# Tzq2doc/distributed_learning_simulator

Hardware: AMD Instinct MI355X
Metric: FL rounds/sec (FedAvg, 100 clients, ResNet-18, CIFAR-10-shaped) (higher is better)
Workload: dtype fp32; 1 GPU; fedavg_resnet18; model=ResNet18, algo=fed_avg, clients=100, local_epochs=5, global_batch=6400, per_client_batch=64, parallelism=client-dp1, backend=hip

## Files before the change

### csrc/bindings.cpp

```cpp
#include <pybind11/pybind11.h>

#include <stdexcept>
#include <string>

#include "dls.h"

namespace py = pybind11;
typedef uintptr_t ptr;

template <typename T>
static T* P(ptr p) {
  return reinterpret_cast<T*>(p);
}
static hipStream_t S(ptr s) { return reinterpret_cast<hipStream_t>(s); }

extern "C" const char* dls_src_hash();

static SgdEpi sgd_arg(const py::object& o) {
  SgdEpi e{};
  if (o.is_none()) return e;
  const py::tuple t = o.cast<py::tuple>();
  if (t.size() != 13) throw std::invalid_argument("sgd epilogue: 13 fields expected");
  e.theta = P<float>(t[0].cast<ptr>());
  e.mom = P<float>(t[1].cast<ptr>());
// ... 37 lines not shown
    p.stats = P<float>(stats);
    p.stats_valid = P<const int>(stats_valid);
    p.f32 = f32;
    p.ldx = ldx;
    p.ldy = ldy;
    p.acc = P<const bf16_t>(acc);
    p.gate = P<const bf16_t>(gate);
    p.x = P<const bf16_t>(x);
    p.w = P<const bf16_t>(w);
    p.y = P<bf16_t>(y);
    p.bias = P<const bf16_t>(bias);
    p.x_cs = x_cs; p.y_cs = y_cs; p.w_cs = w_cs; p.b_cs = b_cs;
    p.B = B; p.H = H; p.W = W; p.C = C; p.OH = OH; p.OW = OW; p.KH = KH; p.KW = KW;
    p.stride = stride; p.pad = pad; p.dil = dil; p.M = M; p.N = N; p.R = R; p.rep = rep; p.relu = relu;
    p.b_kmajor = b_kmajor;
    if (stats && stats_valid && native_option(g_opt_halo_skip, "DLS_SKIP_INVALID", 1)) {
      p.skip_valid = P<const int>(stats_valid);
      p.skip_mul = OH * OW;
    }
    conv_nt(p, K, variant, S(s));
  });
  m.def("conv_dgrad", [](ptr dy, ptr w, ptr dx, ptr acc, long w_cs, int K, int rep, int B, int OH, int OW, int Co, int H,
                         int W, int Ci, int KH, int KW, int stride, int pad, int variant, int f32, ptr s, int ld_dy,
                         long dy_cs, ptr wsplit, long ws_cs, long ws_plane, long x_lo, int acc_compact, ptr bnb_part,
                         ptr bnb_x, long bnb_xld, ptr bnb_y, ptr bnb_mask, ptr bnb_mean, ptr bnb_rstd, ptr bnb_valid,
                         ptr wt_buf, ptr acc_mask, int wt_ready) {
    BNBwdPartials bnb{P<float>(bnb_part), P<const float>(bnb_x), bnb_xld, P<const float>(bnb_y),
                      P<const uint8_t>(bnb_mask), P<const float>(bnb_mean), P<const float>(bnb_rstd),
                      P<const int>(bnb_valid)};
    conv_dgrad(P<const bf16_t>(dy), P<const bf16_t>(w), P<bf16_t>(dx), P<const bf16_t>(acc), w_cs, K, rep, B, OH, OW, Co, H, W, Ci, KH, KW,
               stride, pad, variant, f32, S(s), ld_dy, dy_cs, P<const bf16_t>(wsplit), ws_cs, ws_plane, x_lo, acc_compact,
               bnb_part ? &bnb : nullptr, P<bf16_t>(wt_buf), P<const uint8_t>(acc_mask), wt_ready);
  });
  m.def("wt_planes", [](ptr wsplit, long ws_cs, long ws_plane, ptr wt, int Kw, int Co, int Ci, ptr s) {
    wt_planes(P<const bf16_t>(wsplit), ws_cs, ws_plane, P<bf16_t>(wt), Kw, Co, Ci, S(s));
  });
  m.def("conv_gl_wanted", &conv_gl_wanted);
  m.def("conv_gl_fwd", [](ptr x, ptr w, ptr y, ptr bias, long x_cs, long y_cs, long w_cs, long b_cs, int K, int rep,
                          int B, int H, int W, int C, int OH, int OW, int KH, int KW, int stride, int pad, int N,
                          int relu, ptr s) {
    conv_gl_fwd(P<const bf16_t>(x), P<const bf16_t>(w), P<bf16_t>(y), P<const bf16_t>(bias), x_cs, y_cs, w_cs, b_cs,
                K, rep, B, H, W, C, OH, OW, KH, KW, stride, pad, N, relu, S(s));
  });
  m.def("conv_weight_flip_t", [](ptr w, ptr wt, long w_cs, int Kw, int Co, int KH, int KW, int Ci, ptr s) {
    conv_weight_flip_t(P<const bf16_t>(w), P<bf16_t>(wt), w_cs, Kw, Co, KH, KW, Ci, S(s));
  });
  m.def("conv_gl_dgrad", [](ptr dy, ptr wt, ptr dx, ptr acc, int K, int rep, int B, int OH, int OW, int Co, int H, int W,
                            int Ci, int KH, int KW, int stride, int pad, ptr s) {
    conv_gl_dgrad(P<const bf16_t>(dy), P<const bf16_t>(wt), P<bf16_t>(dx), P<const bf16_t>(acc), K, rep, B, OH, OW, Co, H, W, Ci, KH, KW,
                  stride, pad, S(s));
  });
  m.def("conv_nt_num_variants", &conv_nt_num_variants);
  m.def("conv_nt_default_variant", &conv_nt_default_variant);
  m.def("conv_tn_bn_bwd", [](ptr dy, ptr x, ptr dw, long x_cs, long dw_cs, int B, int H, int W, int C, int OH, int OW,
                             int KH, int KW, int stride, int pad, int M, int Co, int R, int K, int variant, ptr s,
                             int ldx, ptr part, ptr bn_x, ptr bn_mask, ptr bn_coef, ptr bn_valid) {
    ConvTNParams p{};
    p.part = P<float>(part);
    p.f32 = 1;
    p.ldy = Co;
    p.ldx = ldx;
    p.dy = P<const bf16_t>(dy);
    p.x = P<const bf16_t>(x);
    p.dw = P<float>(dw);
    p.dy_cs = (long)M * Co; p.x_cs = x_cs; p.dw_cs = dw_cs;
    p.B = B; p.H = H; p.W = W; p.C = C; p.OH = OH; p.OW = OW; p.KH = KH; p.KW = KW; p.stride = stride; p.pad = pad;
// ... 456 lines not shown
```

### csrc/conv_nt.hip

```cpp
#include "dls.h"
#include "gemm_common.h"

#include <numeric>

namespace {

template <int BM, int BN, int BK, int WM, int WN, int VA, int VB, bool BKM, int DEPTH>
__global__ void __launch_bounds__(WM* WN * 64) conv_nt_kernel(ConvNTParams p) {
  constexpr int T = WM * WN * 64;
  constexpr int TM = BM / (WM * 32);
  constexpr int TN = BN / (WN * 32);
  constexpr int LDA = BK + 8;
  constexpr int KCA = BK / VA, RPA = T / KCA, PA = BM / RPA;
  constexpr int KCB = BK / VB, RPB = T / KCB, PB = BN / RPB;
  constexpr int CCB = BN / VB, RPK = T / CCB, PK = BK / RPK;
  constexpr int LDBK = BN + 32;
  constexpr int NB = BKM ? PK : PB;
  static_assert(PA >= 1 && NB >= 1, "tile too small for thread count");
  static_assert(TM >= 1 && TN >= 1, "wave tile");
  constexpr int NBUF = DEPTH == 0 ? 1 : 2;
  constexpr int B_ROWS = BKM ? BK : BN, B_COLS = BKM ? LDBK : LDA;
  constexpr int A_BYTES = NBUF * BM * LDA * 2, B_BYTES = NBUF * B_ROWS * B_COLS * 2;
  constexpr int SW = TN * 32 + 8;
  constexpr int EPI_BYTES = WM * WN * 32 * SW * 2;
// ... 346 lines not shown
  p.fd_ohw = make_fastdiv((uint32_t)(p.OH * p.OW));
  p.fd_ow = make_fastdiv((uint32_t)p.OW);
  p.fd_kwc = make_fastdiv((uint32_t)(p.KW * p.C));
  p.fd_c = make_fastdiv((uint32_t)p.C);
  if (p.f32) {
    conv_nt_f32(p, K, variant, s);
    return;
  }
  if (p.stats) {
    fprintf(stderr, "conv_nt: epilogue statistics need the fp32 kernels\n");
    abort();
  }
  const bool bkm = p.b_kmajor != 0;
  int va = vec_width(std::gcd(p.C, p.ldx));
  int vb = bkm ? vec_width(p.N) : vec_width(p.R);
  if (va == 1 && vb == 4) vb = 1;
  if (variant < 0) {
    variant = conv_nt_default_variant(p.M, p.N, p.R, p.b_kmajor);
    (void)K;
  }
  const bool w84 = (va == 8 || va == 4) && (vb == 8 || vb == 4);
  if (w84 && !(va == 8 && vb == 8) && !(variant == 0 || variant == 10 || variant == 13 || variant == 6 ||
                                        variant == 7 || variant == 18)) {
    variant = (p.N <= 64) ? 13 : (bkm ? 10 : 0);
  } else if (!w84 && !(variant == 6 || variant == 7 || variant == 18)) {
    variant = (p.N <= 64) ? 7 : 6;
  }
  if (!launch_variant(variant, p, K, va, vb, bkm, s)) fprintf(stderr, "conv_nt: bad variant %d\n", variant);
}

void wt_planes(const bf16_t* wsplit, long ws_cs, long ws_plane, bf16_t* wt, int Kw, int Co, int Ci, hipStream_t s) {
  hipLaunchKernelGGL(wt_planes_kernel, dim3(Kw * 2 * 9, Co / 32, Ci / 32), dim3(256), 0, s, wsplit, ws_cs, ws_plane, wt,
                     Co, Ci);
}

void conv_dgrad(const bf16_t* dy, const bf16_t* w, bf16_t* dx, const bf16_t* acc, long w_cs, int K, int rep, int B, int OH, int OW,
                int Co, int H, int W, int Ci, int KH, int KW, int stride, int pad, int variant, int f32, hipStream_t s,
                int ld_dy, long dy_cs, const bf16_t* wsplit, long ws_cs, long ws_plane, long x_lo, int acc_compact,
                const BNBwdPartials* bnb, bf16_t* wt_buf, const uint8_t* acc_mask, int wt_ready) {
  ConvNTParams p{};
  p.acc_mask = acc_mask;
  if (bnb) {
    if (!f32 || stride != 1 || Ci % 4 != 0 || (bnb->mask && Ci % 8 != 0) || (bnb->xld && bnb->xld % 4 != 0)) {
      fprintf(stderr, "conv_dgrad: BN-backward partials need an fp32 stride-1 dgrad with Ci %% 4 == 0\n");
      abort();
    }
    p.bnb = bnb->part;
    p.bnb_x = bnb->x;
    p.bnb_xld = bnb->xld ? bnb->xld : Ci;
    p.bnb_y = bnb->y;
    p.bnb_mask = bnb->mask;
    p.bnb_mean = bnb->mean;
    p.bnb_rstd = bnb->rstd;
    p.bnb_valid = bnb->valid;
    if (stride == 1 && bnb->valid && native_option(g_opt_halo_skip, "DLS_SKIP_INVALID", 1)) {
      p.skip_valid = bnb->valid;
      p.skip_mul = 1;
    }
  }
  p.x_lo = x_lo;
  p.wsplit = wsplit;
  p.ws_cs = ws_cs;
  p.ws_plane = ws_plane;
  p.f32 = f32;
  p.ldx = ld_dy;
  p.x = dy;
// ... 16 lines not shown
  p.wKH = KH;
  p.wKW = KW;
  p.dil = 1;
  p.stride = 1;
  if (stride == 1) {
    p.OH = H;
    p.OW = W;
    p.KH = KH;
    p.KW = KW;
    p.pad = KH - 1 - pad;
    p.pad_w = KW - 1 - pad;
    p.kh_off = KH - 1;
    p.kw_off = KW - 1;
    p.kh_step = p.kw_step = 1;
    p.out_s = 1;
    p.M = B * H * W;
    p.R = KH * KW * Co;
    if (variant < 0 && !f32 && Ci <= 64 && vec_width(Ci) == 8 && vec_width(Co) == 8) variant = 14;
    if (wt_buf && f32 && x_lo != 0 && wsplit && KH == 3 && KW == 3 && pad == 1 && Co % 32 == 0 && Ci % 32 == 0) {
      const int Kw = K / rep;
      if (!wt_ready)
        hipLaunchKernelGGL(wt_planes_kernel, dim3(Kw * 2 * 9, Co / 32, Ci / 32), dim3(256), 0, s, wsplit, ws_cs,
                           ws_plane, wt_buf, Co, Ci);
      p.b_kmajor = 0;
      p.wsplit = wt_buf;
      p.ws_cs = 2L * 9 * Ci * Co;
      p.ws_plane = 9L * Ci * Co;
      p.w = wt_buf;
      p.w_cs = p.ws_cs;
    }
    conv_nt(p, K, variant, s);
    return;
  }
  for (int ph = 0; ph < stride; ++ph) {
    const int Hc = (H - ph + stride - 1) / stride;
    if (Hc <= 0) continue;
    const int kh0 = (ph + pad) % stride;
    const int nkh = kh0 < KH ? (KH - kh0 + stride - 1) / stride : 0;
    const int dh = (ph + pad - kh0) / stride;
    for (int pw = 0; pw < stride; ++pw) {
      const int Wc = (W - pw + stride - 1) / stride;
      if (Wc <= 0) continue;
      const int kw0 = (pw + pad) % stride;
      const int nkw = kw0 < KW ? (KW - kw0 + stride - 1) / stride : 0;
      const int dw = (pw + pad - kw0) / stride;
      ConvNTParams q = p;
      q.OH = Hc;
      q.OW = Wc;
      q.M = B * Hc * Wc;
      if (acc_compact) {
        q.acc = (ph == 0 && pw == 0) ? acc : nullptr;
        q.acc_compact = 1;
        q.acc_cs = (long)B * Hc * Wc * Ci;
      }
      q.out_s = stride;
      q.out_ph = ph;
      q.out_pw = pw;
      q.out_H = H;
      q.out_W = W;
      if (nkh == 0 || nkw == 0) {
        q.KH = q.KW = 1;
        q.R = 0;
        q.pad = q.pad_w = 0;
        q.kh_off = q.kw_off = 0;
        q.kh_step = q.kw_step = 1;
      } else {
// ... 14 lines not shown
```

### csrc/dls.h

```cpp
#pragma once
#include <hip/hip_runtime.h>
#include <stdint.h>

typedef uint16_t bf16_t;

constexpr int kOptUnset = -1000000;
extern int g_opt_attn_mfma, g_opt_conv_gl, g_opt_pl_min_wg;
extern int g_opt_halo_wgrad_unroll;
extern int g_opt_halo_skip;
extern int g_opt_conv_pix;
int native_option(int& slot, const char* env, int dflt);
bool set_native_option(const char* name, int value);

struct FastDiv {
  uint32_t d, mul, shift;
};

static inline FastDiv make_fastdiv(uint32_t d) {
  FastDiv f;
  f.d = d;
  uint32_t s = 0;
  while ((1u << s) < d) ++s;
  f.shift = s;
  f.mul = (uint32_t)((((uint64_t)1 << 32) * (((uint64_t)1 << s) - d)) / d + 1);
  return f;
}

__device__ __forceinline__ uint32_t fdiv(uint32_t n, const FastDiv& f) {
  return (__umulhi(n, f.mul) + n) >> f.shift;
}

struct ConvNTParams {
  const bf16_t* x;
  const bf16_t* w;
  bf16_t* y;
  const bf16_t* bias;
  const bf16_t* acc;
  long acc_cs;
  int acc_compact;
  const uint8_t* acc_mask;
  const bf16_t* gate;
  long x_cs, y_cs, w_cs, b_cs;
  int B, H, W, C;
// ... 173 lines not shown
void conv_gl_fwd(const bf16_t* x, const bf16_t* w, bf16_t* y, const bf16_t* bias, long x_cs, long y_cs, long w_cs,
                 long b_cs, int K, int rep, int B, int H, int W, int C, int OH, int OW, int KH, int KW, int stride,
                 int pad, int N, int relu, hipStream_t s);
void conv_weight_flip_t(const bf16_t* w, bf16_t* wt, long w_cs, int Kw, int Co, int KH, int KW, int Ci,
                        hipStream_t s);
void conv_gl_dgrad(const bf16_t* dy, const bf16_t* wt, bf16_t* dx, const bf16_t* acc, int K, int rep, int B, int OH, int OW, int Co,
                   int H, int W, int Ci, int KH, int KW, int stride, int pad, hipStream_t s);

void conv_nt(ConvNTParams p, int K, int variant, hipStream_t s);
int conv_nt_num_variants();
int conv_nt_default_variant(int M, int N, int R, int b_kmajor);
void conv_dgrad(const bf16_t* dy, const bf16_t* w, bf16_t* dx, const bf16_t* acc, long w_cs, int K, int rep, int B, int OH, int OW,
                int Co, int H, int W, int Ci, int KH, int KW, int stride, int pad, int variant, int f32, hipStream_t s,
                int ld_dy = 0, long dy_cs = 0, const bf16_t* wsplit = nullptr, long ws_cs = 0, long ws_plane = 0,
                long x_lo = 0, int acc_compact = 0,
                const BNBwdPartials* bnb = nullptr,
                bf16_t* wt_buf = nullptr,
                const uint8_t* acc_mask = nullptr,
                int wt_ready = 0);
void wt_planes(const bf16_t* wsplit, long ws_cs, long ws_plane, bf16_t* wt, int Kw, int Co, int Ci, hipStream_t s);
void conv_tn(ConvTNParams p, int K, int variant, hipStream_t s);
int conv_tn_num_variants();
int conv_tn_splitk(int K, int Co, int R, int M, int C, int variant, int f32, int ldy = 0, int ldx = 0,
                   int planes = 0);
void conv_nt_f32(const ConvNTParams& p, int K, int variant, hipStream_t s);
int conv_nt_f32_num_variants();
void conv_tn_f32(ConvTNParams p, int K, int variant, hipStream_t s);
bool conv_nt_pl_supported(const ConvNTParams& p);
bool conv_nt_pl(const ConvNTParams& p, int K, int variant, hipStream_t s);
int conv_nt_pl_num_variants();
int conv_nt_pl_variant();
void conv_nt_pl_set_variant(int v);
bool conv_halo(const ConvNTParams& p, int K, hipStream_t s);
bool conv_halo_bn_supported(int B, int H, int W, int C, int N);
void bn_coef_sums(const double* sums, long sums_cs, int ldp, const float* gamma, const float* beta,
                  const int* valid_rows, long g_cs, int K, int R, int C, float eps, int rep, float* mean, float* rstd,
                  float* coef, hipStream_t s);
void part_sum_f64(const float* part, int K, int nparts, int g, double* out, long out_cs, int ldo, hipStream_t s);
long chan_sums_f64_ws(int R, int C);
void chan_sums_f64(const float* x, long x_cs, int ldx, int K, int R, int C, const int* valid, double* ws, double* out,
                   long out_cs, int ldo, hipStream_t s);
void bn_apply_only(const float* x, const float* coef, const int* valid_rows, int K, int R, int C, int relu,
                   bf16_t* yp, uint8_t* rmask, hipStream_t s, float* y = nullptr);
bool conv_halo_bn_fwd(const float* x, long x_cs, const float* coef, int relu, const int* valid_rows,
                      const bf16_t* wsplit, long ws_cs, long ws_plane, int rep, float* y, long y_cs, int K, int B,
                      int H, int W, int C, int N, float* stats, const int* stats_valid, hipStream_t s,
                      bf16_t* yp = nullptr, uint8_t* mask = nullptr);
bool conv_halo_bn_dense_supported(int B, int H, int W, int C, int N);
bool conv_halo_bn_dense_fwd(const float* x, long x_cs, int ldx, int creal, const float* coef, int relu,
                            const int* valid_rows, const bf16_t* wsplit, long ws_cs, long ws_plane, int rep, float* y,
                            long y_cs, int ldy, int K, int B, int H, int W, int C, int N, float* stats,
                            const int* stats_valid, float* ny, long ny_cs, int ldny, uint8_t* mask, hipStream_t s);
bool dense_dgrad_supported(int B, int H, int W, int C, int N);
long dense_dgrad_ws_floats(int K, int B, int H, int C);
bool dense_dgrad_bn(DenseDgradParams p, const float* gamma, long g_cs, float* dgamma, float* dbeta, long dg_cs,
                    float* ws, hipStream_t s);
void bn_bwd_coef_parts(const float* part, int nparts, const float* gamma, long g_cs, const int* valid_rows,
                       const float* mean, const float* rstd, int K, int R, int C, float* coef, float* dgamma,
                       float* dbeta, long dg_cs, hipStream_t s);
bool dense_wgrad_supported(int B, int H, int W, int C, int N);
long dense_wgrad_part_floats(int K, int B, int H, int W, int C);
bool dense_wgrad(const float* dy, long dy_cs, int ldy, const float* y, long y_cs, float* dw, long dw_cs, float* part,
                 int K, int B, int H, int W, int C, int N, hipStream_t s, const float* bn_sc = nullptr,
                 int ldy_x = 0, const int* valid_rows = nullptr);
void conv_halo_set_mode(int m);
void conv_halo_set_variant(int v);
// ... 204 lines not shown
```

### csrc/elementwise.hip

```cpp
#include <algorithm>

#include "common.h"
#include "sgd_epi.h"
#include "dls.h"
#include <cstdlib>
#include <cstring>
#include <stdexcept>

namespace {

template <typename T>
__global__ void pool_fwd_kernel(const T* __restrict__ x, T* __restrict__ y, int* __restrict__ idx,
                                long total, int H, int W, int C, int OH, int OW, int k, int stride, int pad,
                                int mode) {
  const long i = (long)blockIdx.x * blockDim.x + threadIdx.x;
  if (i >= total) return;
  const int c = i % C;
  long t = i / C;
  const int ow = t % OW;
  t /= OW;
  const int oh = t % OH;
  const long img = t / OH;
  const T* xi = x + img * H * W * C;
  float best = -INFINITY, acc = 0.f;
// ... 1118 lines not shown
  const dim3 grid((unsigned)std::min<long>(cdiv(total, 256), 4096), K);
  if (f32)
    hipLaunchKernelGGL(dropout_apply_kernel<float>, grid, dim3(256), 0, s, static_cast<const float*>(x),
                       static_cast<float*>(out), rows, N, ld, seeds, p, scale);
  else
    hipLaunchKernelGGL(dropout_apply_kernel<bf16_t>, grid, dim3(256), 0, s, static_cast<const bf16_t*>(x),
                       static_cast<bf16_t*>(out), rows, N, ld, seeds, p, scale);
}

long dropout_planes_ws_floats(int K, long rows, int N) { return (long)K * cdiv(rows, DP_RB) * N; }

void dropout_planes(const float* x, float* out, bf16_t* yp, int K, long rows, int N, const uint32_t* seeds, float p,
                    float scale, hipStream_t s, float* colsum, long colsum_cs, float* ws) {
  if (rows == 0 || K == 0) return;
  if (N % 2) throw std::runtime_error("dropout_planes: N must be even");
  const dim3 grid((unsigned)cdiv(rows, DP_RB), K);
  hipLaunchKernelGGL(dropout_planes_kernel, grid, dim3(256), 0, s, x, out, yp, rows, N, seeds, p, scale,
                     colsum ? ws : nullptr);
  if (colsum) fold_col_partials(ws, (int)grid.x, N, colsum, colsum_cs, K, s);
}

void synth_images(const int64_t* idx, long n, long npix, int C, int Cout, const int* source, const float* proto,
                  unsigned long long salt, float sqrt6, float noise, float* out, hipStream_t s) {
  const long total = n * (npix / C) * Cout;
  if (total == 0) return;
  hipLaunchKernelGGL(synth_images_kernel, dim3((unsigned)std::min<long>(cdiv(total, 256), 65536)), dim3(256), 0, s,
                     idx, n, npix, C, Cout, source, proto, salt, sqrt6, noise, out);
}

int g_opt_attn_mfma = kOptUnset, g_opt_conv_gl = kOptUnset;
int g_opt_pl_min_wg = kOptUnset;
int g_opt_halo_wgrad_unroll = kOptUnset, g_opt_halo_skip = kOptUnset;
int g_opt_conv_pix = kOptUnset;

int native_option(int& slot, const char* env, int dflt) {
  if (slot == kOptUnset) {
    const char* e = getenv(env);
    slot = e ? atoi(e) : dflt;
  }
  return slot;
}

bool set_native_option(const char* name, int value) {
  struct Entry {
    const char* name;
    int* slot;
  };
  const Entry table[] = {{"attn_mfma", &g_opt_attn_mfma},
                         {"conv_gl", &g_opt_conv_gl},       {"pl_min_wg", &g_opt_pl_min_wg},
                         {"halo_wgrad_unroll", &g_opt_halo_wgrad_unroll}, {"halo_skip", &g_opt_halo_skip},
                         {"conv_pix", &g_opt_conv_pix}};
  for (const Entry& t : table)
    if (strcmp(t.name, name) == 0) {
      *t.slot = value;
      return true;
    }
  return false;
}
```

### distributed_learning_simulator_amd/ops/hip.py

```python

from __future__ import annotations

import collections
import importlib
import os
import threading

import torch

from ..options import OPTIONS
from . import ref

try:
    _C = importlib.import_module("distributed_learning_simulator_amd._dls_hip")
except ImportError as e:
    raise ImportError(
        "HIP extension _dls_hip is not built; run `python -m distributed_learning_simulator_amd.ops.build` "
        f"(original error: {e})"
    ) from e


def _check_provenance() -> None:
    from . import build as _build

# ... 248 lines not shown
        assert bnb is None
        if acc_mask is not None:
            from .functional import MaskedGrad

            acc, acc_mask = MaskedGrad(acc, acc_mask).dense(), None
        if acc_compact:
            full = torch.zeros((K, B, H, W, Ci), dtype=dy.dtype, device=dy.device)
            full[:, :, ::stride, ::stride] = acc
            acc, acc_compact = full, False
        dx = torch.empty((K, B, H, W, Ci), dtype=dy.dtype, device=dy.device)
        for b0, b1 in _batch_chunks(B, per_sample):
            dx[:, b0:b1] = conv_dgrad(dy[:, b0:b1], w, in_hw, stride, pad,
                                      acc=None if acc is None else acc[:, b0:b1].contiguous(), w_split=w_split)
        return dx
    dy, ld_dy = _pix_stride(dy)
    f32 = _f32(dy)
    _check(w, dy.dtype, contiguous=False, name="w")
    assert Co2 == Co
    w_cs, rep = _client_view(w, K)
    dx = torch.empty((K, B, H, W, Ci), dtype=dy.dtype, device=dy.device)
    if acc is not None and not acc_compact:
        assert acc.shape == dx.shape and acc.dtype == dy.dtype and acc.is_contiguous(), acc.shape
    if (not f32 and not acc_compact and ld_dy == Co and (stride == 1 or (gl_mode == 1 and acc is None))
            and _gl(K, B * H * W, Ci, Co, KH * KW)):
        wt = torch.empty((Kw, Ci, KH, KW, Co), dtype=BF16, device=dy.device)
        _C.conv_weight_flip_t(_p(w), _p(wt), w.stride(0), Kw, Co, KH, KW, Ci, _s())
        _C.conv_gl_dgrad(_p(dy), _p(wt), _p(dx), _p(acc), K, rep, B, OH, OW, Co, H, W, Ci, KH, KW, stride, pad, _s())
        return dx
    ws_p, ws_cs, ws_plane = _wsplit_args(w_split if f32 else None, w)
    dyp, dy_cs, dy_lo = _p(dy), dy.stride(0), 0
    if dy_planes is not None and ws_p and planes_ok(Co, Ci, ld_dy):
        dyp, dy_cs, dy_lo = _planes_args(dy_planes, dy)
        planes_launches["dgrad"] += 1
    wt_ready = wt_buf is not None
    if (wt or wt_ready) and _wt_dgrad_ok(Co, Ci, KH, KW, H, W, stride, pad, bool(dy_lo), ws_p):
        if wt_buf is None:
            wt_buf = torch.empty(Kw * 2 * 9 * Ci * Co, dtype=BF16, device=dy.device)
        planes_launches["dgrad_wt"] += 1
    else:
        assert not wt_ready, "conv_dgrad: a prebuilt wt_buf for a dgrad that does not take it"
        wt_buf = None
    _C.conv_dgrad(dyp, _p(w), _p(dx), _p(acc), w_cs, K, rep, B, OH, OW, Co, H, W, Ci, KH, KW, stride, pad,
                  nt_f32_variant if f32 else nt_variant, f32, _s(), ld_dy, dy_cs, ws_p, ws_cs, ws_plane, dy_lo,
                  int(bool(acc_compact)), *bnb_args, _p(wt_buf), _p(acc_mask), int(wt_ready))
    return dx


_part_cache: dict = {}


def _tn_part(numel: int, device) -> torch.Tensor:
    return _grown(_part_cache, (device, torch.cuda.current_stream().cuda_stream), numel, device)


def _sgd_arg(sgd):
    if sgd is None:
        return None
    f, _, off = sgd
    wd, mom, damp, nest = f.hyper
    assert f.theta.stride(1) == 1 and f.mom.stride(0) == f.theta.stride(0) and f.split.is_contiguous()
    return (_p(f.theta) + off * 4, _p(f.mom) + off * 4, _p(f.split) + off * 2, f.theta.stride(0), f.split.stride(0),
            f.split.stride(1), _p(f.lr), _p(f.active), _p(f.first), float(wd), float(mom), float(damp), int(nest))


def _tn_launch(dy, x, gw, dy_cs, x_cs, B, H, W, C, OH, OW, KH, KW, stride, pad, M, Co, R, K, f32, ldy, ldx,
               dy_planes=None, x_planes=None, sgd=None):
    planes = f32 and dy_planes is not None and x_planes is not None
    tv = (_C.conv_tn_pl_variant() if planes else tn_f32_variant) if f32 else tn_variant
    dyp, xp, dy_lo, x_lo = _p(dy), _p(x), 0, 0
    if planes:
        dyp, dy_cs, dy_lo = _planes_args(dy_planes, dy)
        xp, x_cs, x_lo = _planes_args(x_planes, x)
        planes_launches["wgrad"] += 1
    splitk = _C.conv_tn_splitk(K, Co, R, M, C, tv, f32, ldy, ldx, int(planes))
    part = NULL
    if splitk > 1:
# ... 1465 lines not shown
```

### distributed_learning_simulator_amd/options.py

```python

from __future__ import annotations

import contextlib
import dataclasses
import os
import threading


def _env_bool(name: str, default: bool) -> bool:
    v = os.environ.get(name)
    return default if v is None else v not in ("0", "", "false", "False")


def _env_int(name: str, default: int) -> int:
    v = os.environ.get(name)
    return default if v is None or v == "" else int(v)


@dataclasses.dataclass
class RuntimeOptions:
    planes: bool = dataclasses.field(default_factory=lambda: _env_bool("DLS_PLANES", True))
    """BatchNorms emit bf16 (hi, lo) planes for the LDS-DMA plane / halo GEMMs (off: every conv
    splits its operand in registers)."""
    fused_sgd: bool = dataclasses.field(default_factory=lambda: _env_bool("DLS_FUSED_SGD", True))
    """SGD steps of the weights whose plane / halo wgrad kernels can apply them (csrc/sgd_epi.h)
    run in those kernels; the flat step covers the rest (engine.params.FusedSGD)."""
    tfm_planes: bool = dataclasses.field(default_factory=lambda: _env_bool("DLS_TFM_PLANES", True))
    """Transformer split-plane producers: the FFN hidden activation and its gradient (linear1 /
    linear2 epilogues) and the dropout backward of the residual-branch linears (out_proj /
    linear2) write planes for the plane GEMMs (off: fp32 only). (Attention outputs writing planes
    measured +0.4-0.5 s per FedOBD stage-1 round each, profiles/r5_c6_ab_tfm_planes.txt: removed.)"""
    bn_bwd_parts: bool = dataclasses.field(default_factory=lambda: _env_bool("DLS_BN_BWD_PARTS", True))
    """BN backward partial sums from the consuming conv's dgrad epilogue (off: own reduction)."""
    bn_fused_halo: bool = dataclasses.field(default_factory=lambda: _env_bool("DLS_BN_FUSED_HALO", True))
    """A BN(+ReLU) whose only reader is a 3x3 stride-1 conv (ResNet BasicBlock bn1) is applied in
    that conv's halo loader (ops.functional DeferredBN; off: BN apply pass + plane conv)."""
    bn_res_fold: bool = dataclasses.field(default_factory=lambda: _env_bool("DLS_BN_RES_FOLD", True))
    """A ResNet downsample shortcut's BN is applied inside the block's last BN apply, which reads
    its raw input as the residual (ops.functional DeferredRes; off: its own apply pass)."""
    bn_stem_defer: bool = dataclasses.field(default_factory=lambda: _env_bool("DLS_BN_STEM_DEFER", True))
    """The CIFAR ResNet stem BN(+ReLU), read by layer1.0.conv1 (planes) and by layer1.0.bn2 (fp32, as
    its identity residual), is applied by those two readers: the conv in its halo loader, the BN
    in its residual fold (ops.functional DeferredStemBN; off: one apply pass writes both forms)."""
    dense_bn_halo: bool = dataclasses.field(default_factory=lambda: _env_bool("DLS_DENSE_BN_HALO", True))
    """DenseNet growth convs apply their BN + ReLU in the halo loader over the block buffer's
    channel prefix (off: BN apply pass + implicit-GEMM conv)."""
    halo_wgrad: bool = dataclasses.field(default_factory=lambda: _env_bool("DLS_HALO_WGRAD", True))
    """3x3 stride-1 weight gradients of 64-512-channel convs (ResNet layers 1-3) on the LDS-halo
    kernel (csrc/conv_halo_wgrad.hip; off: the implicit-GEMM TN kernel)."""
    bn_bwd_in_wgrad: bool = dataclasses.field(default_factory=lambda: _env_bool("DLS_BN_BWD_IN_WGRAD", True))
    """A training BN(+ReLU) whose input gradient feeds only a 3x3 stride-1 conv's backward (ResNet
    BasicBlock bn1 / identity-block bn2, layers 1-3) computes its coefficients only: that conv's halo
    weight gradient applies the BN backward in its dY loader and writes dX's planes for the dgrad
    (ops.functional DeferredBNBwd; off: the BN backward's own apply pass writes them)."""
    bn_bwd_in_wgrad_f32: bool = dataclasses.field(default_factory=lambda: _env_bool("DLS_BN_BWD_IN_WGRAD_F32", True))
    """A training BN(+ReLU) behind a conv whose input needs no gradient (the ResNet stem) computes
    its backward coefficients only: the conv's fp32 weight gradient applies the BN backward in its dY
    loader (ops.functional DeferredBNBwdF32, csrc/conv_f32.hip; off: the BN backward's own apply pass
    writes dX and the weight gradient reads it back)."""
    dense_wgrad_halo: bool = dataclasses.field(default_factory=lambda: _env_bool("DLS_DENSE_WGRAD_HALO", True))
    """DenseNet growth-conv weight gradients on the LDS-halo kernel (the normalised prefix staged
    once per pixel tile for all nine taps; off: the implicit-GEMM TN kernel)."""
    dense_dgrad_fused: bool = dataclasses.field(default_factory=lambda: _env_bool("DLS_DENSE_DGRAD_FUSED", True))
    """DenseNet growth-conv input gradients fused with the BN backward (csrc/conv_dense_dgrad.hip:
    dX̂ recomputed in a sums pass and an apply pass instead of stored and read twice; off: the
    implicit-GEMM dgrad + the BN backward passes)."""
    dense_y_recompute: bool = dataclasses.field(default_factory=lambda: _env_bool("DLS_DENSE_Y_RECOMPUTE", True))
    """With the fused dgrad and the halo weight gradient, DenseNet training stores no normalised
    activation: both backward kernels rebuild relu(BN(x)) from the raw prefix and the forward's
    (scale, shift), bitwise (off: the forward's halo conv writes it for them)."""
    dense_stats_cache: bool = dataclasses.field(default_factory=lambda: _env_bool("DLS_DENSE_STATS_CACHE", True))
    """DenseNet blocks (fused growth convs) sum each channel's statistics once, from the producing
    conv's epilogue, into running fp64 sums the BN coefficients read (off: a statistics pass over
    the prefix per layer)."""
    deterministic: bool = dataclasses.field(default_factory=lambda: _env_bool("DLS_DETERMINISTIC", True))
    """Split-K weight gradients and column sums folded in a fixed order (off: fp32 atomics)."""
    streams: int = dataclasses.field(default_factory=lambda: _env_int("DLS_STREAMS", 2))
    """Sub-cohort HIP streams trained concurrently on one GPU."""
    ragged_steps: bool = dataclasses.field(default_factory=lambda: _env_bool("DLS_RAGGED_STEPS", True))
    """A cohort's clients are ordered by shard size, so in an epoch's last steps (where only the
    clients with the largest shards still have a batch) the active clients are a row prefix and
    the step runs those rows only (off: every step runs all K rows, idle ones masked)."""
# ... 26 lines not shown


_NATIVE_UNSET = -1000000


def _push_native(native: dict) -> None:
    if not native:
        return
    try:
        from .ops import hip
    except ImportError:
        return
    for k, v in native.items():
        hip._C.set_native_option(str(k), _NATIVE_UNSET if v is None else int(v))


def update(**kw) -> dict:
    old = {}
    for k, v in kw.items():
        if k not in _FIELDS:
            raise KeyError(f"unknown runtime option {k!r}; known: {sorted(_FIELDS)}")
        old[k] = getattr(OPTIONS, k)
        if k == "native":
            merged = dict(OPTIONS.native)
            merged.update(v or {})
            v = {n: x for n, x in merged.items() if x is not None}
        else:
            v = type(old[k])(v)
        setattr(OPTIONS, k, v)
    if "native" in kw:
        _push_native(kw["native"] or {})
    if "skip_invalid" in kw:
        _push_native({"halo_skip": int(OPTIONS.skip_invalid)})
    return old


def _restore(old: dict, kw: dict) -> None:
    old = dict(old)
    native_prev = old.pop("native", None)
    for k, v in old.items():
        setattr(OPTIONS, k, v)
    if native_prev is not None:
        update(native={n: native_prev.get(n) for n in (kw.get("native") or {})})


@contextlib.contextmanager
def override(**kw):
    old = update(**kw)
    try:
        yield OPTIONS
    finally:
        _restore(old, kw)


def config_options(config) -> dict:
    extra = getattr(config, "extra", None) or {}
    return dict(extra.get("runtime_options") or {})


_scope_lock = threading.Lock()
_scope = {"count": 0, "opts": None, "saved": None}


@contextlib.contextmanager
def scoped(opts: dict | None):
    opts = dict(opts or {})
    with _scope_lock:
        if _scope["count"] and opts != _scope["opts"]:
            raise RuntimeError(f"concurrent runs with different runtime_options: {opts} vs {_scope['opts']}")
        if _scope["count"] == 0:
            _scope["saved"] = update(**opts) if opts else {}
            _scope["opts"] = opts
        _scope["count"] += 1
    try:
# ... 14 lines not shown
```

Measured before the change: 0.3069 rounds/s.

## Add LDS-halo stride-2 dgrad kernel covering all four parity classes in one launch

Adds a new HIP kernel for 3x3 stride-2 input gradients on split bf16 planes. It stages the dY halo in LDS once and computes all four output parity classes with MFMA, replacing four separate parity-class implicit-GEMM launches. The goal is less redundant dY traffic and fewer launches for the ResNet layer2.0 and layer3.0 conv1 dgrad. It brings a large new kernel with narrow shape gates and a runtime option, on by default.

```diff
diff --git a/csrc/bindings.cpp b/csrc/bindings.cpp
--- a/csrc/bindings.cpp
+++ b/csrc/bindings.cpp
@@ -93,6 +93,7 @@
                stride, pad, variant, f32, S(s), ld_dy, dy_cs, P<const bf16_t>(wsplit), ws_cs, ws_plane, x_lo, acc_compact,
                bnb_part ? &bnb : nullptr, P<bf16_t>(wt_buf), P<const uint8_t>(acc_mask), wt_ready);
   });
+  m.def("conv_dgrad_takes_s2", &conv_dgrad_takes_s2);
   m.def("wt_planes", [](ptr wsplit, long ws_cs, long ws_plane, ptr wt, int Kw, int Co, int Ci, ptr s) {
     wt_planes(P<const bf16_t>(wsplit), ws_cs, ws_plane, P<bf16_t>(wt), Kw, Co, Ci, S(s));
   });
diff --git a/csrc/conv_halo_s2.hip b/csrc/conv_halo_s2.hip
--- /dev/null
+++ b/csrc/conv_halo_s2.hip
@@ -0,0 +1,299 @@
+#include "dls.h"
+#include "gemm_common.h"
+
+namespace {
+
+typedef __attribute__((address_space(3))) void lds_void;
+typedef uint32_t u32x2 __attribute__((ext_vector_type(2)));
+
+__device__ __forceinline__ void sdma16(__amdgpu_buffer_rsrc_t r, unsigned char* lds, uint32_t off) {
+  __builtin_amdgcn_raw_ptr_buffer_load_lds(r, (lds_void*)lds, 16, off, 0, 0, 0);
+}
+
+template <int N>
+__device__ __forceinline__ void swait_vm() {
+  static_assert(N >= 0 && N < 64, "vmcnt range");
+  __builtin_amdgcn_s_waitcnt((N & 15) | ((N >> 4) << 14) | (7 << 4) | (15 << 8));
+}
+
+struct S2DgradParams {
+  const bf16_t* dy;
+  const bf16_t* wsplit;
+  float* dx;
+  const float* acc;
+  long dy_cs, dy_lo, ws_cs, ws_plane;
+  int B, OH, OW, Co, Ci, rep;
+};
+
+struct S2Tap {
+  int cls, kh2, kw2;
+};
+__host__ __device__ constexpr S2Tap s2_tap(int t9) {
+  const int cls = t9 == 0 ? 0 : t9 < 3 ? 1 : t9 < 5 ? 2 : 3;
+  const int j = t9 - (cls == 0 ? 0 : cls == 1 ? 1 : cls == 2 ? 3 : 5);
+  return S2Tap{cls, cls == 3 ? j >> 1 : cls == 2 ? j : 0, (cls & 1) ? j & 1 : 0};
+}
+
+template <int IMG, int TH, int TW, int WM, int WN, int NCH, int NBS>
+__global__ void __launch_bounds__(WM* WN * 64) conv_halo_s2_dgrad_kernel(S2DgradParams p) {
+  constexpr int NW = WM * WN, BM = WM * 32, BN = WN * 32;
+  static_assert(BM == IMG * TH * TW, "one 32-row tile per wave row");
+  static_assert(TW == 4 || TW == 8 || TW == 16, "halo pitch TW + 4, key factor 3");
+  constexpr int HH2 = TH + 1, HW2 = TW + 2, PITCH = TW + 4, KC = 3;
+  constexpr int HP = IMG * HH2 * PITCH;
+  constexpr int HG = (HP + 15) / 16;
+  constexpr int HI = (HG + NW - 1) / NW;
+  constexpr int H_PL = HG * 1024;
+  constexpr int B_PL = BN * 64;
+  constexpr int NBI = BN / 16;
+  constexpr int GB = 2 * NBI / NW;
+  static_assert(GB >= 1 && GB * NW == 2 * NBI, "weight DMA split");
+  constexpr int D = NBS - 1;
+  static_assert(D >= 1 && (D - 1) * GB < 64, "ring depth");
+  constexpr int B_OFF = NCH * 2 * H_PL;
+  constexpr int SMEM = B_OFF + NBS * 2 * B_PL;
+  static_assert(SMEM <= 160 * 1024, "LDS");
+  __shared__ __attribute__((aligned(1024))) unsigned char smem[SMEM];
+
+  const int lane = threadIdx.x & 63;
+  const int wid = __builtin_amdgcn_readfirstlane(threadIdx.x >> 6);
+  const int H = 2 * p.OH, W = 2 * p.OW, N = p.Ci;
+  const int tpi = p.OH / TH;
+  const int tilesM = IMG == 1 ? p.B * tpi : (p.B + IMG - 1) / IMG;
+  const int bid = xcd_remap(blockIdx.x, gridDim.x);
+  const int client = bid / tilesM;
+  const int tm = bid - client * tilesM;
+  const int b0 = IMG == 1 ? tm / tpi : tm * IMG;
+  const int h0 = IMG == 1 ? (tm % tpi) * TH : 0;
+
+  const long a_img = (long)p.B * p.OH * p.OW * p.Co;
+  const auto ar = make_rsrc(p.dy + (long)client * p.dy_cs, (uint32_t)((p.dy_lo + a_img) * 2));
+  const uint32_t a_lo = (uint32_t)(p.dy_lo * 2);
+  const long wkhwn = 9L * N;
+  const auto br = make_rsrc(p.wsplit + (long)(client / p.rep) * p.ws_cs, (uint32_t)((p.ws_plane + p.Co * wkhwn) * 2));
+  const uint32_t b_lo = (uint32_t)(p.ws_plane * 2);
+  const int nch = p.Co / 32, tilesN = (N + BN - 1) / BN;
+
+#pragma unroll
+  for (int i = 0; i < HI; ++i) {
+    const int grp = i * NW + wid;
+    if (grp >= HG) continue;
+    const int hr = grp * 16 + (lane >> 2);
+    const int img = hr / (HH2 * PITCH), rem = hr - img * (HH2 * PITCH);
+    const int hh = rem / PITCH, ww = rem - hh * PITCH;
+    const int ih = h0 + hh, iw = ww - 1;
+    const int lc = (lane & 3) ^ (((hr >> 2) + (hr / PITCH) * KC) & 3);
+    const bool ok = hr < HP && ww < HW2 && b0 + img < p.B && ih < p.OH && (unsigned)iw < (unsigned)p.OW;
+    const int off = (((b0 + img) * p.OH + ih) * p.OW + iw) * p.Co + lc * 8;
+    for (int c = 0; c < nch; ++c) {
+      unsigned char* d = smem + (c * 2) * H_PL + grp * 1024;
+      const uint32_t o = (uint32_t)(off + c * 32) * 2u;
+      sdma16(ar, d, ok ? o : OOB_OFF);
+      sdma16(ar, d + H_PL, ok ? o + a_lo : OOB_OFF);
+    }
+  }
+  constexpr int CPR = BN / 8, RPI = 64 / CPR;
+  constexpr int SD = (128 / BN) > 1 ? 128 / BN : 1, SS = (BN / 32) < 4 ? BN / 32 : 4;
+  int b_src[GB], b_n[GB], b_dst[GB];
+#pragma unroll
+  for (int i = 0; i < GB; ++i) {
+    const int j = i * NW + wid, plane = j / NBI, idx = j - plane * NBI;
+    const int kr = idx * RPI + lane / CPR;
+    const int f = SS > 1 ? (kr / SD) & (SS - 1) : 0;
+    b_n[i] = ((lane % CPR) ^ (f << 2)) * 8;
+    b_src[i] = (int)(kr * wkhwn) + b_n[i];
+    b_dst[i] = plane * B_PL + idx * 1024;
+  }
+  int i_nt = 0, i_t9 = 0, i_c = 0, i_slot = 0;
+  auto issue_next = [&]() {
+    const S2Tap t = s2_tap(i_t9);
+    const int kh = (t.cls >> 1) ? 2 - 2 * t.kh2 : 1, kw = (t.cls & 1) ? 2 - 2 * t.kw2 : 1;
+    const int boff = (int)(i_c * 32 * wkhwn) + (kh * 3 + kw) * N + i_nt * BN;
+    const bool live = i_nt < tilesN;
+    unsigned char* Bs = smem + B_OFF + i_slot * 2 * B_PL;
+#pragma unroll
+    for (int i = 0; i < GB; ++i) {
+      const int j = i * NW + wid;
+      const bool ok = live && i_nt * BN + b_n[i] < N;
+      const uint32_t off = (uint32_t)(b_src[i] + boff) * 2u + (j >= NBI ? b_lo : 0u);
+      sdma16(br, Bs + b_dst[i], ok ? off : OOB_OFF);
+    }
+    if (++i_c == nch) {
+      i_c = 0;
+      if (++i_t9 == 9) {
+        i_t9 = 0;
+        ++i_nt;
+      }
+    }
+    if (++i_slot == NBS) i_slot = 0;
+  };
+#pragma unroll
+  for (int d = 0; d < D; ++d) issue_next();
+
+  const int wm0 = (wid / WN) * 32, wn0 = (wid % WN) * 32;
+  const int g = lane >> 4, q = (lane >> 2) & 3, pp = lane & 3, h = lane >> 5;
+  int hbase, hkey;
+  {
+    const int pix = wm0 + (lane & 31);
+    const int img = pix / (TH * TW), rr = pix - img * (TH * TW);
+    const int th = rr / TW, tw = rr - th * TW;
+    hbase = img * HH2 * PITCH + th * PITCH + tw;
+    hkey = (img * HH2 + th) * KC;
+  }
+  f32x16 acc[4];
+  auto compute = [&](f32x16& a4, int c, int slot, int dh, int dw) {
+    const unsigned char* Hs = smem + (c * 2) * H_PL;
+    const unsigned char* Bs = smem + B_OFF + slot * 2 * B_PL;
+    const int hr = hbase + dh * PITCH + dw;
+    u32x2 bq[2][4];
+    uint32_t baddr[2];
+#pragma unroll
+    for (int ks = 0; ks < 2; ++ks) {
+      const int kr = ks * 16 + 8 * h + q;
+      const int f = SS > 1 ? (kr / SD) & (SS - 1) : 0;
+      const int col = (wn0 + 16 * (g & 1) + 4 * pp) ^ (f << 5);
+      baddr[ks] = (uint32_t)(uintptr_t)(lds_void*)(Bs + (kr * BN + col) * 2);
+    }
+    asm volatile(
+        "ds_read_b64_tr_b16 %0, %8\n\t"
+        "ds_read_b64_tr_b16 %1, %8 offset:%10\n\t"
+        "ds_read_b64_tr_b16 %2, %8 offset:%11\n\t"
+        "ds_read_b64_tr_b16 %3, %8 offset:%12\n\t"
+        "ds_read_b64_tr_b16 %4, %9\n\t"
+        "ds_read_b64_tr_b16 %5, %9 offset:%10\n\t"
+        "ds_read_b64_tr_b16 %6, %9 offset:%11\n\t"
+        "ds_read_b64_tr_b16 %7, %9 offset:%12\n\t"
+        "s_waitcnt lgkmcnt(0)"
+        : "=&v"(bq[0][0]), "=&v"(bq[0][1]), "=&v"(bq[0][2]), "=&v"(bq[0][3]), "=&v"(bq[1][0]), "=&v"(bq[1][1]),
+          "=&v"(bq[1][2]), "=&v"(bq[1][3])
+        : "v"(baddr[0]), "v"(baddr[1]), "n"(4 * BN * 2), "n"(B_PL), "n"(B_PL + 4 * BN * 2)
+        : "memory");
+#pragma unroll
+    for (int ks = 0; ks < 2; ++ks) {
+      const unsigned char* a = Hs + hr * 64 + (((ks * 2 + h) ^ (((hr >> 2) + hkey + dh * KC) & 3)) << 4);
+      const bf16x8 ah = *reinterpret_cast<const bf16x8*>(a);
+      const bf16x8 al = *reinterpret_cast<const bf16x8*>(a + H_PL);
+      const bf16x8 bh = __builtin_shufflevector(__builtin_bit_cast(bf16x4, bq[ks][0]),
+                                                __builtin_bit_cast(bf16x4, bq[ks][1]), 0, 1, 2, 3, 4, 5, 6, 7);
+      const bf16x8 bl = __builtin_shufflevector(__builtin_bit_cast(bf16x4, bq[ks][2]),
+                                                __builtin_bit_cast(bf16x4, bq[ks][3]), 0, 1, 2, 3, 4, 5, 6, 7);
+      a4 = __builtin_amdgcn_mfma_f32_32x32x16_bf16(al, bh, a4, 0, 0, 0);
+      a4 = __builtin_amdgcn_mfma_f32_32x32x16_bf16(ah, bl, a4, 0, 0, 0);
+      a4 = __builtin_amdgcn_mfma_f32_32x32x16_bf16(ah, bh, a4, 0, 0, 0);
+    }
+  };
+
+  static_assert((TW == 16 && TH == 8 && IMG == 1) || (TW == 8 && TH == 4 && IMG == 1) ||
+                    (TW == 4 && TH == 4 && IMG == 2),
+                "carry-free split of the accumulator rows");
+  const auto yr = make_rsrc(p.dx + (long)client * p.B * H * W * N, (uint32_t)((long)p.B * H * W * N * 4));
+  const auto cr = make_rsrc(p.acc ? p.acc + (long)client * p.B * p.OH * p.OW * N : p.dx,
+                            p.acc ? (uint32_t)((long)p.B * p.OH * p.OW * N * 4) : 0u);
+  const int l_th = (wm0 + 4 * h) / TW, l_tw = (wm0 + 4 * h) % TW;
+  auto store_class = [&](const f32x16& a4, int nt, int cls) {
+    const int ph = cls >> 1, pw = cls & 1;
+    const int n = nt * BN + wn0 + (lane & 31);
+    const bool addc = p.acc != nullptr && cls == 0;
+    const uint32_t vy =
+        n < N ? (uint32_t)((((b0 * H + 2 * (h0 + l_th) + ph) * W + 2 * l_tw + pw) * N + n) * 4) : OOB_OFF;
+    const uint32_t vc =
+        n < N ? (uint32_t)((((b0 * p.OH + h0 + l_th) * p.OW + l_tw) * N + n) * 4) : OOB_OFF;
+    float av[16];
+#pragma unroll
+    for (int e = 0; e < 16; ++e) {
+      const int ep = 8 * (e >> 2);
+      const int d_tw = (e & 3) + ep % TW, d_th = (ep / TW) % TH, d_img = ep / TW / TH;
+      av[e] = 0.f;
+      if (addc && b0 + d_img < p.B)
+        av[e] = __uint_as_float(__builtin_amdgcn_raw_buffer_load_b32(
+            cr, vc, (uint32_t)(((d_img * p.OH + d_th) * p.OW + d_tw) * N * 4), 0));
+    }
+#pragma unroll
+    for (int e = 0; e < 16; ++e) {
+      const int ep = 8 * (e >> 2);
+      const int d_tw = (e & 3) + ep % TW, d_th = (ep / TW) % TH, d_img = ep / TW / TH;
+      if (b0 + d_img < p.B) {
+        float v = a4[e];
+        if (addc) v += av[e];
+        __builtin_amdgcn_raw_buffer_store_b32(__float_as_uint(v), yr, vy,
+                                              (uint32_t)(((d_img * H + 2 * d_th) * W + 2 * d_tw) * N * 4), 0);
+      }
+    }
+  };
+
+  int slot = 0;
+  for (int nt = 0; nt < tilesN; ++nt) {
+#pragma unroll
+    for (int k = 0; k < 4; ++k) acc[k] = f32x16{};
+#pragma unroll
+    for (int t9 = 0; t9 < 9; ++t9) {
+      constexpr S2Tap taps[9] = {s2_tap(0), s2_tap(1), s2_tap(2), s2_tap(3), s2_tap(4),
+                                 s2_tap(5), s2_tap(6), s2_tap(7), s2_tap(8)};
+      for (int c = 0; c < nch; ++c) {
+        swait_vm<(D - 1) * GB>();
+        __builtin_amdgcn_s_barrier();
+        issue_next();
+        compute(acc[taps[t9].cls], c, slot, taps[t9].kh2, 1 + taps[t9].kw2);
+        if (++slot == NBS) slot = 0;
+      }
+    }
+#pragma unroll
+    for (int k = 0; k < 4; ++k) store_class(acc[k], nt, k);
+    swait_vm<0>();
+  }
+}
+
+template <int IMG, int TH, int TW, int WM, int WN, int NCH, int NBS>
+void launch_s2(const S2DgradParams& p, int K, hipStream_t s) {
+  const int tilesM = IMG == 1 ? p.B * (p.OH / TH) : cdiv(p.B, IMG);
+  hipLaunchKernelGGL((conv_halo_s2_dgrad_kernel<IMG, TH, TW, WM, WN, NCH, NBS>), dim3(K * tilesM),
+                     dim3(WM * WN * 64), 0, s, p);
+}
+
+int s2_config(int B, int OH, int OW, int Co, int H, int W, int Ci, bool any) {
+  if (H != 2 * OH || W != 2 * OW || Co % 32 || Ci % 32 || B < 1) return -1;
+  if (OW == 16 && OH % 8 == 0 && Co <= 128) return 0;
+  if (OW == 8 && OH % 4 == 0 && Co <= (any ? 256 : 128)) return 1;
+  if (OW == 4 && OH == 4 && Co <= 256) return 2;
+  return -1;
+}
+
+}
+
+bool conv_halo_s2_dgrad_supported(int B, int OH, int OW, int Co, int H, int W, int Ci) {
+  const int opt = native_option(g_opt_halo_s2_dgrad, "DLS_HALO_S2_DGRAD", 1);
+  if (opt == 0 || conv_nt_pl_variant() >= 0) return false;
+  if (s2_config(B, OH, OW, Co, H, W, Ci, opt == 2) < 0) return false;
+  return (long)B * OH * OW * Co * 4 < (long)OOB_OFF && (long)Co * 9 * Ci * 4 < (long)OOB_OFF &&
+         (long)B * H * W * Ci * 4 < (long)OOB_OFF;
+}
+
+bool conv_halo_s2_dgrad(const bf16_t* dy, long dy_cs, long dy_lo, const bf16_t* wsplit, long ws_cs, long ws_plane,
+                        float* dx, const float* acc, int K, int rep, int B, int OH, int OW, int Co, int H, int W,
+                        int Ci, hipStream_t s) {
+  if (!conv_halo_s2_dgrad_supported(B, OH, OW, Co, H, W, Ci) || dy_lo == 0 || wsplit == nullptr) return false;
+  if ((dy_lo + (long)B * OH * OW * Co) * 2 >= (long)OOB_OFF || (ws_plane + (long)Co * 9 * Ci) * 2 >= (long)OOB_OFF)
+    return false;
+  S2DgradParams p{};
+  p.dy = dy;
+  p.wsplit = wsplit;
+  p.dx = dx;
+  p.acc = acc;
+  p.dy_cs = dy_cs;
+  p.dy_lo = dy_lo;
+  p.ws_cs = ws_cs;
+  p.ws_plane = ws_plane;
+  p.B = B;
+  p.OH = OH;
+  p.OW = OW;
+  p.Co = Co;
+  p.Ci = Ci;
+  p.rep = rep;
+  switch (s2_config(B, OH, OW, Co, H, W, Ci, g_opt_halo_s2_dgrad == 2)) {
+    case 0: launch_s2<1, 8, 16, 4, 2, 4, 8>(p, K, s); break;
+    case 1: launch_s2<1, 4, 8, 1, 4, 8, 6>(p, K, s); break;
+    case 2: launch_s2<2, 4, 4, 1, 4, 8, 4>(p, K, s); break;
+    default: return false;
+  }
+  return true;
+}
diff --git a/csrc/conv_nt.hip b/csrc/conv_nt.hip
--- a/csrc/conv_nt.hip
+++ b/csrc/conv_nt.hip
@@ -402,6 +402,14 @@
 void wt_planes(const bf16_t* wsplit, long ws_cs, long ws_plane, bf16_t* wt, int Kw, int Co, int Ci, hipStream_t s) {
   hipLaunchKernelGGL(wt_planes_kernel, dim3(Kw * 2 * 9, Co / 32, Ci / 32), dim3(256), 0, s, wsplit, ws_cs, ws_plane, wt,
                      Co, Ci);
+}
+
+bool conv_dgrad_takes_s2(int f32, int planes, int has_acc, int acc_compact, int has_bnb, int has_mask, int variant,
+                         int ld_dy, int B, int OH, int OW, int Co, int H, int W, int Ci, int KH, int KW, int stride,
+                         int pad) {
+  if (!f32 || !planes || stride != 2 || KH != 3 || KW != 3 || pad != 1 || variant >= 0) return false;
+  if ((has_acc && !acc_compact) || has_bnb || has_mask || (ld_dy != 0 && ld_dy != Co)) return false;
+  return conv_halo_s2_dgrad_supported(B, OH, OW, Co, H, W, Ci);
 }
 
 void conv_dgrad(const bf16_t* dy, const bf16_t* w, bf16_t* dx, const bf16_t* acc, long w_cs, int K, int rep, int B, int OH, int OW,
@@ -484,6 +492,11 @@
     conv_nt(p, K, variant, s);
     return;
   }
+  if (conv_dgrad_takes_s2(f32, x_lo != 0 && wsplit != nullptr, acc != nullptr, acc_compact, bnb != nullptr,
+                          acc_mask != nullptr, variant, ld_dy, B, OH, OW, Co, H, W, Ci, KH, KW, stride, pad) &&
+      conv_halo_s2_dgrad(dy, p.x_cs, x_lo, wsplit, ws_cs, ws_plane, reinterpret_cast<float*>(dx),
+                         reinterpret_cast<const float*>(acc), K, rep, B, OH, OW, Co, H, W, Ci, s))
+    return;
   for (int ph = 0; ph < stride; ++ph) {
     const int Hc = (H - ph + stride - 1) / stride;
     if (Hc <= 0) continue;
diff --git a/csrc/dls.h b/csrc/dls.h
--- a/csrc/dls.h
+++ b/csrc/dls.h
@@ -9,6 +9,7 @@
 extern int g_opt_halo_wgrad_unroll;
 extern int g_opt_halo_skip;
 extern int g_opt_conv_pix;
+extern int g_opt_halo_s2_dgrad;
 int native_option(int& slot, const char* env, int dflt);
 bool set_native_option(const char* name, int value);
 
@@ -248,6 +249,13 @@
 int conv_nt_pl_variant();
 void conv_nt_pl_set_variant(int v);
 bool conv_halo(const ConvNTParams& p, int K, hipStream_t s);
+bool conv_halo_s2_dgrad_supported(int B, int OH, int OW, int Co, int H, int W, int Ci);
+bool conv_halo_s2_dgrad(const bf16_t* dy, long dy_cs, long dy_lo, const bf16_t* wsplit, long ws_cs, long ws_plane,
+                        float* dx, const float* acc, int K, int rep, int B, int OH, int OW, int Co, int H, int W,
+                        int Ci, hipStream_t s);
+bool conv_dgrad_takes_s2(int f32, int planes, int has_acc, int acc_compact, int has_bnb, int has_mask, int variant,
+                         int ld_dy, int B, int OH, int OW, int Co, int H, int W, int Ci, int KH, int KW, int stride,
+                         int pad);
 bool conv_halo_bn_supported(int B, int H, int W, int C, int N);
 void bn_coef_sums(const double* sums, long sums_cs, int ldp, const float* gamma, const float* beta,
                   const int* valid_rows, long g_cs, int K, int R, int C, float eps, int rep, float* mean, float* rstd,
diff --git a/csrc/elementwise.hip b/csrc/elementwise.hip
--- a/csrc/elementwise.hip
+++ b/csrc/elementwise.hip
@@ -1174,6 +1174,7 @@
 int g_opt_pl_min_wg = kOptUnset;
 int g_opt_halo_wgrad_unroll = kOptUnset, g_opt_halo_skip = kOptUnset;
 int g_opt_conv_pix = kOptUnset;
+int g_opt_halo_s2_dgrad = kOptUnset;
 
 int native_option(int& slot, const char* env, int dflt) {
   if (slot == kOptUnset) {
@@ -1191,7 +1192,7 @@
   const Entry table[] = {{"attn_mfma", &g_opt_attn_mfma},
                          {"conv_gl", &g_opt_conv_gl},       {"pl_min_wg", &g_opt_pl_min_wg},
                          {"halo_wgrad_unroll", &g_opt_halo_wgrad_unroll}, {"halo_skip", &g_opt_halo_skip},
-                         {"conv_pix", &g_opt_conv_pix}};
+                         {"conv_pix", &g_opt_conv_pix},     {"halo_s2_dgrad", &g_opt_halo_s2_dgrad}};
   for (const Entry& t : table)
     if (strcmp(t.name, name) == 0) {
       *t.slot = value;
diff --git a/distributed_learning_simulator_amd/ops/hip.py b/distributed_learning_simulator_amd/ops/hip.py
--- a/distributed_learning_simulator_amd/ops/hip.py
+++ b/distributed_learning_simulator_amd/ops/hip.py
@@ -304,6 +304,11 @@
     if dy_planes is not None and ws_p and planes_ok(Co, Ci, ld_dy):
         dyp, dy_cs, dy_lo = _planes_args(dy_planes, dy)
         planes_launches["dgrad"] += 1
+    variant = nt_f32_variant if f32 else nt_variant
+    if stride == 2 and _C.conv_dgrad_takes_s2(f32, int(bool(dy_lo and ws_p)), int(acc is not None), int(bool(acc_compact)),
+                                              int(bnb is not None), int(acc_mask is not None), variant, ld_dy, B, OH,
+                                              OW, Co, H, W, Ci, KH, KW, stride, pad):
+        planes_launches["dgrad_s2"] += 1
     wt_ready = wt_buf is not None
     if (wt or wt_ready) and _wt_dgrad_ok(Co, Ci, KH, KW, H, W, stride, pad, bool(dy_lo), ws_p):
         if wt_buf is None:
@@ -313,7 +318,7 @@
         assert not wt_ready, "conv_dgrad: a prebuilt wt_buf for a dgrad that does not take it"
         wt_buf = None
     _C.conv_dgrad(dyp, _p(w), _p(dx), _p(acc), w_cs, K, rep, B, OH, OW, Co, H, W, Ci, KH, KW, stride, pad,
-                  nt_f32_variant if f32 else nt_variant, f32, _s(), ld_dy, dy_cs, ws_p, ws_cs, ws_plane, dy_lo,
+                  variant, f32, _s(), ld_dy, dy_cs, ws_p, ws_cs, ws_plane, dy_lo,
                   int(bool(acc_compact)), *bnb_args, _p(wt_buf), _p(acc_mask), int(wt_ready))
     return dx
 
diff --git a/distributed_learning_simulator_amd/options.py b/distributed_learning_simulator_amd/options.py
--- a/distributed_learning_simulator_amd/options.py
+++ b/distributed_learning_simulator_amd/options.py
@@ -48,6 +48,10 @@
     halo_wgrad: bool = dataclasses.field(default_factory=lambda: _env_bool("DLS_HALO_WGRAD", True))
     """3x3 stride-1 weight gradients of 64-512-channel convs (ResNet layers 1-3) on the LDS-halo
     kernel (csrc/conv_halo_wgrad.hip; off: the implicit-GEMM TN kernel)."""
+    halo_s2_dgrad: bool = dataclasses.field(default_factory=lambda: _env_bool("DLS_HALO_S2_DGRAD", True))
+    """3x3 stride-2 input gradients on split planes (ResNet layer2.0 / layer3.0 conv1) run as one
+    LDS-halo launch that stages dY once for all four parity classes (csrc/conv_halo_s2.hip; off: four
+    parity-class implicit GEMMs). Bitwise the same dX either way."""
     bn_bwd_in_wgrad: bool = dataclasses.field(default_factory=lambda: _env_bool("DLS_BN_BWD_IN_WGRAD", True))
     """A training BN(+ReLU) whose input gradient feeds only a 3x3 stride-1 conv's backward (ResNet
     BasicBlock bn1 / identity-block bn2, layers 1-3) computes its coefficients only: that conv's halo
@@ -140,6 +144,8 @@
         _push_native(kw["native"] or {})
     if "skip_invalid" in kw:
         _push_native({"halo_skip": int(OPTIONS.skip_invalid)})
+    if "halo_s2_dgrad" in kw:
+        _push_native({"halo_s2_dgrad": int(OPTIONS.halo_s2_dgrad)})
     return old
 
 
@@ -148,6 +154,8 @@
     native_prev = old.pop("native", None)
     for k, v in old.items():
         setattr(OPTIONS, k, v)
+    if "halo_s2_dgrad" in old:
+        _push_native({"halo_s2_dgrad": int(OPTIONS.halo_s2_dgrad)})
     if native_prev is not None:
         update(native={n: native_prev.get(n) for n in (kw.get("native") or {})})
 
```

After: 0.3087 rounds/s (median of 6 runs). About the same (+0.6%).
